# paritybit-ai/XFL

Hardware: AMD Instinct MI355X
Metric: 2048-bit Paillier encrypts/s (device-resident) (higher is better)
Workload: dtype u32; 1 GPU; DJN private-key (CRT) encrypt, obfuscated, precision 7, 1000000 float64 plaintexts/GPU resident in HBM; key_bits=2048, elements_per_gpu=1000000, fixed_base_window_bits=23, fixed_base_window_split=False, parallelism=shard1, table_bytes=193273528320

## Files before the change

### __graft_entry__.py

```python
import os
import sys

ROOT = os.path.dirname(os.path.abspath(__file__))
if ROOT not in sys.path:
    sys.path.insert(0, ROOT)


def build() -> None:
    from xfl_amd import build as b
    b.build()
    from oracle import build as ob
    ob.build()
    import runpy
    try:
        runpy.run_path(os.path.join(ROOT, "tests", "native", "build.py"), run_name="tests_native_build")["build"]()
    except Exception as exc:
        print(f"warning: device self-test harnesses not built: {exc}", file=sys.stderr)
    import xfl_amd
    from xfl_amd import _native
    _native.lib()


def smoke() -> None:
    import numpy as np

    from oracle import paillier_oracle as O
    from xfl_amd import _native as nat
    from xfl_amd.paillier.utils import getprimeover
    import random
    import math

    rng = random.Random(7)
    while True:
        p, q = getprimeover(1024, rng=rng), getprimeover(1024, rng=rng)
        if p != q and math.gcd(p - 1, q - 1) == 2:
            break
    n = p * q
    x = rng.getrandbits(n.bit_length()) | (1 << (n.bit_length() - 1))
    h = pow(-(x * x), n, n * n)
    dk = nat.DeviceKey(2048, n, p, q, h, device=0)
    ok = O.derive_private(p, q, h)
    vals = np.random.default_rng(0).standard_normal(64) * 10
    ms = [O.encode_element(ok, float(v), 7)[0] for v in vals]
    rs = [rng.randrange(1, ok["djn_exp_bound"]) for _ in vals]
    ct = nat.words_to_ints(dk.encrypt_words(nat.ints_to_words(ms, dk.nw), nat.ints_to_words(rs, dk.rand_words)))
    want = [O.encrypt_m(ok, m, r) for m, r in zip(ms, rs)]
    assert ct == want, "HIP encrypt differs from the oracle"
    back = nat.words_to_ints(dk.decrypt_words(nat.ints_to_words(ct, dk.n2w)))
    assert back == ms, "HIP decrypt differs from the oracle"
    print("smoke ok: 64 DJN-CRT encryptions + decryptions bit-exact vs oracle on cuda:0")


if __name__ == "__main__":
    build()
    if "--smoke" in sys.argv:
        smoke()
```

### xfl_amd/csrc/bn_dev.hpp

```cpp
#pragma once
#include <hip/hip_runtime.h>
#include <stdint.h>

namespace xhe {

#define XHE_DEV __device__ __forceinline__
#define XHE_INL __attribute__((always_inline))

#ifndef XHE_SQ_ACC
#define XHE_SQ_ACC 2
#endif
XHE_DEV uint64_t mad64(uint32_t a, uint32_t b, uint64_t c) {
  asm("v_mad_u64_u32 %0, vcc, %1, %2, %0" : "+v"(c) : "v"(a), "v"(b) : "vcc");
  return c;
}
template <int N>
XHE_DEV void mad_shift(uint64_t (&T)[N], const uint32_t (&b)[N], uint32_t a) {
  int j = 1;
#pragma unroll
  for (; j + 6 <= N; j += 6)
    asm("v_mad_u64_u32 %0, vcc, %7, %8, %1\n\t"
        "v_mad_u64_u32 %1, vcc, %7, %9, %2\n\t"
        "v_mad_u64_u32 %2, vcc, %7, %10, %3\n\t"
        "v_mad_u64_u32 %3, vcc, %7, %11, %4\n\t"
// ... 325 lines not shown
    for (int k = 0; k < 8; ++k) nb[0][k] = R.f[k];
    x0 = mad64s(m, R.n0, x0);
    mac4v(T, b, ai, m, 1, R.h);
    advance();
#pragma unroll
    for (int blk = 0; blk < (J8 - 5) / 8; ++blk) {
      const int j = 5 + 8 * blk;
      const int cur = blk & 1;
      if (j + 16 <= J8) {
        asm volatile("" ::"s"(nb[cur][0]), "s"(nb[cur][1]), "s"(nb[cur][2]), "s"(nb[cur][3]), "s"(nb[cur][4]),
                     "s"(nb[cur][5]), "s"(nb[cur][6]), "s"(nb[cur][7]));
        __builtin_amdgcn_sched_barrier(0);
#pragma unroll
        for (int k = 0; k < 8; ++k) nb[cur ^ 1][k] = Np[j + 8 + k];
        __builtin_amdgcn_sched_barrier(0);
      }
      mac8v(T, b, ai, m, j, nb[cur]);
      if (stage < 4) advance();
      else __builtin_amdgcn_sched_barrier(0);
    }
    if constexpr (TL >= 4) mac4v(T, b, ai, m, J8, R.t);
#pragma unroll
    for (int k = (TL >= 4 ? 4 : 0); k < TL; ++k) T[J8 + k - 1] = mad64s(m, R.t[k], mad64(ai, b[J8 + k], T[J8 + k]));
#pragma unroll
    for (int k = 0; k < 4; ++k)
      if (stage < 4) advance();
    T[L - 1] = 0;
    x0 = xn;
    m = mn;
  }

  XHE_DEV void red4v(uint64_t (&T)[L], uint32_t m, int j, const uint32_t* n) const {
    asm("v_mad_u64_u32 %0, vcc, %5, %6, %1\n\t"
        "v_mad_u64_u32 %1, vcc, %5, %7, %2\n\t"
        "v_mad_u64_u32 %2, vcc, %5, %8, %3\n\t"
        "v_mad_u64_u32 %3, vcc, %5, %9, %4"
        : "+v"(T[j - 1]), "+v"(T[j]), "+v"(T[j + 1]), "+v"(T[j + 2])
        : "v"(T[j + 3]), "v"(m), "s"(n[0]), "s"(n[1]), "s"(n[2]), "s"(n[3])
        : "vcc");
  }
  XHE_DEV void red8v(uint64_t (&T)[L], uint32_t m, int j, const uint32_t* n) const {
    asm("v_mad_u64_u32 %0, vcc, %9, %10, %1\n\t"
        "v_mad_u64_u32 %1, vcc, %9, %11, %2\n\t"
        "v_mad_u64_u32 %2, vcc, %9, %12, %3\n\t"
        "v_mad_u64_u32 %3, vcc, %9, %13, %4\n\t"
        "v_mad_u64_u32 %4, vcc, %9, %14, %5\n\t"
        "v_mad_u64_u32 %5, vcc, %9, %15, %6\n\t"
        "v_mad_u64_u32 %6, vcc, %9, %16, %7\n\t"
        "v_mad_u64_u32 %7, vcc, %9, %17, %8"
        : "+v"(T[j - 1]), "+v"(T[j]), "+v"(T[j + 1]), "+v"(T[j + 2]), "+v"(T[j + 3]), "+v"(T[j + 4]),
          "+v"(T[j + 5]), "+v"(T[j + 6])
        : "v"(T[j + 7]), "v"(m), "s"(n[0]), "s"(n[1]), "s"(n[2]), "s"(n[3]), "s"(n[4]), "s"(n[5]), "s"(n[6]),
          "s"(n[7])
        : "vcc");
  }
  XHE_DEV void step1_red(const uint32_t* Np, const NRes& R, uint64_t (&T)[L], uint32_t hi_i, uint32_t& m,
                         uint64_t& x0) const {
    uint64_t xn = 0;
    uint32_t t = 0, mn = 0;
    int stage = 0;
    auto advance = [&]() XHE_INL {
      if (stage == 0) {
        T[0] += x0 >> W;
        asm volatile("" : "+v"(T[0]));
      } else if (stage == 1) {
        xn = T[0];
      } else if (stage == 2) {
        t = (uint32_t)xn * n0inv;
        asm volatile("" : "+v"(t));
      } else if (stage == 3) {
        mn = t & MASK;
        asm volatile("" : "+v"(mn));
      }
      ++stage;
      __builtin_amdgcn_sched_barrier(0);
    };
    uint32_t nb[2][8];
#pragma unroll
    for (int k = 0; k < 8; ++k) nb[0][k] = R.f[k];
    x0 = mad64s(m, R.n0, x0);
    red4v(T, m, 1, R.h);
    advance();
#pragma unroll
    for (int blk = 0; blk < (J8 - 5) / 8; ++blk) {
      const int j = 5 + 8 * blk;
      const int cur = blk & 1;
      if (j + 16 <= J8) {
        asm volatile("" ::"s"(nb[cur][0]), "s"(nb[cur][1]), "s"(nb[cur][2]), "s"(nb[cur][3]), "s"(nb[cur][4]),
                     "s"(nb[cur][5]), "s"(nb[cur][6]), "s"(nb[cur][7]));
        __builtin_amdgcn_sched_barrier(0);
#pragma unroll
        for (int k = 0; k < 8; ++k) nb[cur ^ 1][k] = Np[j + 8 + k];
        __builtin_amdgcn_sched_barrier(0);
      }
      red8v(T, m, j, nb[cur]);
      if (stage < 4) advance();
      else __builtin_amdgcn_sched_barrier(0);
    }
    if constexpr (TL >= 4) red4v(T, m, J8, R.t);
#pragma unroll
    for (int k = (TL >= 4 ? 4 : 0); k < TL; ++k) T[J8 + k - 1] = mad64s(m, R.t[k], T[J8 + k]);
#pragma unroll
    for (int k = 0; k < 4; ++k)
      if (stage < 4) advance();
    T[L - 1] = hi_i;
    x0 = xn;
    m = mn;
  }
  template <int C>
  XHE_DEV uint64_t sq_column(const uint32_t (&a)[L], uint64_t carry) const {
    constexpr int lo = C - (S - 1) > 0 ? C - (S - 1) : 0;
    uint64_t s[XHE_SQ_ACC] = {};
#pragma unroll
    for (int i = lo; 2 * i < C; ++i) s[(i - lo) % XHE_SQ_ACC] = mad64(a[i], a[C - i], s[(i - lo) % XHE_SQ_ACC]);
#pragma unroll
    for (int k = 1; k < XHE_SQ_ACC; ++k) s[0] += s[k];
    uint64_t x = (s[0] << 1) + carry;
    if constexpr ((C & 1) == 0) x = mad64(a[C / 2], a[C / 2], x);
    return x;
  }
  template <int C, class HI>
  XHE_DEV void sq_columns(const uint32_t (&a)[L], uint32_t (&lo)[L], uint64_t carry, uint4& q, const HI& hi) const {
    if constexpr (C < 2 * S) {
      const uint64_t x = C < 2 * S - 1 ? sq_column<C < 2 * S - 1 ? C : 0>(a, carry) : carry;
      const uint32_t limb = (uint32_t)x & MASK;
      if constexpr (C < S) {
        lo[C] = limb;
      } else {
        constexpr int h = C - S;
        if constexpr ((h & 3) == 0) q.x = limb;
        else if constexpr ((h & 3) == 1) q.y = limb;
        else if constexpr ((h & 3) == 2) q.z = limb;
        else q.w = limb;
        if constexpr ((h & 3) == 3 || C == 2 * S - 1) {
          if constexpr ((h & 3) < 3) q.w = 0;
          if constexpr ((h & 3) < 2) q.z = 0;
          if constexpr ((h & 3) < 1) q.y = 0;
          hi.put4(h >> 2, q);
        }
      }
      sq_columns<C + 1, HI>(a, lo, x >> W, q, hi);
    }
  }
  static constexpr bool kSqr = TPI == 1 && L >= 13;
  template <class HI>
  XHE_DEV void sqr(uint32_t (&b)[L], const HI& hi) const {
    uint32_t lo[L];
    uint4 q = make_uint4(0u, 0u, 0u, 0u);
    sq_columns<0, HI>(b, lo, 0ull, q, hi);
    uint64_t T[L];
#pragma unroll
    for (int j = 0; j < L; ++j) T[j] = lo[j];
    hi.sync();
    const uint32_t* Np = np();
    NRes R;
    load_res(Np, R);
    uint64_t x0 = T[0];
    uint32_t m = ((uint32_t)x0 * n0inv) & MASK;
    uint4 cur = hi.load4(0);
    int i = 0;
    for (; i + 4 <= S; i += 4) {
      uint4 nxt = hi.load4(i + 4 < S4 ? i + 4 : i);
      __builtin_amdgcn_sched_barrier(0);
      step1_red(Np, R, T, cur.x, m, x0);
      __builtin_amdgcn_sched_barrier(0);
      step1_red(Np, R, T, cur.y, m, x0);
      __builtin_amdgcn_sched_barrier(0);
      step1_red(Np, R, T, cur.z, m, x0);
      __builtin_amdgcn_sched_barrier(0);
      step1_red(Np, R, T, cur.w, m, x0);
      __builtin_amdgcn_sched_barrier(0);
      cur = nxt;
    }
#pragma unroll
    for (int r = 0; r < (S & 3); ++r) step1_red(Np, R, T, comp4(cur, r), m, x0);
    normalize(T, b);
  }

  XHE_DEV void step(const uint32_t* Np, uint64_t (&T)[L], const uint32_t (&b)[L], uint32_t ai, uint32_t ai_next,
                    uint32_t& m, uint64_t& x0, bool lead) const {
    static_assert(L >= 5, "pipelined step needs L >= 5");
    uint64_t xn = 0;
    uint32_t t = 0, mn = 0;
    int stage = 0;
    auto advance = [&]() XHE_INL {
      if (stage == 0) {
        T[0] += x0 >> W;
        asm volatile("" : "+v"(T[0]));
      } else if (stage == 1) {
        xn = mad64(ai_next, b[0], T[0]);
        asm volatile("" : "+v"(xn));
      } else if (stage == 2) {
        t = (uint32_t)xn * n0inv;
        asm volatile("" : "+v"(t));
      } else if (stage == 3) {
        mn = G::bcast0(t & MASK);
        asm volatile("" : "+v"(mn));
      }
      ++stage;
      __builtin_amdgcn_sched_barrier(0);
    };
    x0 = madN(Np, m, 0, x0);
    mac4(Np, T, b, ai, m, 1);
    advance();
    int j = 5;
#pragma unroll
    for (; j + 8 <= L; j += 8) {
      mac8(Np, T, b, ai, m, j);
      if (stage < 4) advance();
    }
#pragma unroll
    for (; j + 4 <= L; j += 4) {
      mac4(Np, T, b, ai, m, j);
      if (stage < 4) advance();
    }
#pragma unroll
    for (; j < L; ++j) T[j - 1] = madN(Np, m, j, mad64(ai, b[j], T[j]));
#pragma unroll
    for (int k = 0; k < 4; ++k)
      if (stage < 4) advance();
    T[L - 1] = (uint64_t)G::from_next((uint32_t)x0 & MASK);
    x0 = xn;
    m = mn;
  }

  XHE_DEV void normalize(const uint64_t (&T)[L], uint32_t (&b)[L]) const {
    uint64_t c = 0;
#pragma unroll
    for (int j = 0; j < L; ++j) {
      uint64_t x = T[j] + c;
      b[j] = (uint32_t)x & MASK;
      c = x >> W;
      __builtin_amdgcn_sched_barrier(0);
    }
    if constexpr (TPI >= 4) {
      uint64_t cin = G::from_prev64(c);
      uint32_t all = 1u;
#pragma unroll
      for (int j = 0; j < L; ++j) {
        uint64_t x = (uint64_t)b[j] + cin;
        b[j] = (uint32_t)x & MASK;
        cin = x >> W;
        all &= (b[j] == MASK) ? 1u : 0u;
        __builtin_amdgcn_sched_barrier(0);
      }
      constexpr uint64_t top = TPI == 16 ? 0x8000800080008000ull : TPI == 8 ? 0x8080808080808080ull
                                                                            : 0x8888888888888888ull;
      const uint64_t gm = __builtin_amdgcn_ballot_w64(cin != 0) & ~top;
      const uint64_t tm = (gm | __builtin_amdgcn_ballot_w64(all != 0)) & ~top;
      const uint64_t cm = (gm + tm) ^ gm ^ tm;
      uint32_t ci = (uint32_t)(cm >> (threadIdx.x & 63)) & 1u;
#pragma unroll
      for (int j = 0; j < L; ++j) {
        uint32_t x = b[j] + ci;
        b[j] = x & MASK;
        ci = x >> W;
      }
    } else if constexpr (TPI > 1) {
#pragma unroll
      for (int r = 1; r < TPI; ++r) {
        uint64_t cin = G::from_prev64(c);
#pragma unroll
        for (int j = 0; j < L; ++j) {
          uint64_t x = (uint64_t)b[j] + cin;
          b[j] = (uint32_t)x & MASK;
          cin = x >> W;
          __builtin_amdgcn_sched_barrier(0);
        }
        c = cin;
      }
    }
  }

  template <class A>
  XHE_DEV void mul(uint32_t (&b)[L], const A& a) const {
    uint64_t T[L];
#pragma unroll
    for (int j = 0; j < L; ++j) T[j] = 0;
    run<A>(T, b, a);
    normalize(T, b);
  }

  template <class A>
  XHE_DEV void run(uint64_t (&T)[L], const uint32_t (&b)[L], const A& a) const {
    const bool lead = G::g() == 0;
    const uint32_t* Np = np();
    uint4 cur = a.load4(0);
    uint64_t x0 = mad64(cur.x, b[0], T[0]);
    uint32_t m = G::bcast0(((uint32_t)x0 * n0inv) & MASK);
    int i = 0;
    if constexpr (TPI == 1 && L >= 13) {
      NRes R;
      load_res(Np, R);
      for (; i + 4 <= S; i += 4) {
        uint4 nxt = a.load4(i + 4 < S4 ? i + 4 : i);
        __builtin_amdgcn_sched_barrier(0);
        step1(Np, R, T, b, cur.x, cur.y, m, x0, lead);
        __builtin_amdgcn_sched_barrier(0);
        step1(Np, R, T, b, cur.y, cur.z, m, x0, lead);
        __builtin_amdgcn_sched_barrier(0);
        step1(Np, R, T, b, cur.z, cur.w, m, x0, lead);
        __builtin_amdgcn_sched_barrier(0);
        step1(Np, R, T, b, cur.w, nxt.x, m, x0, lead);
        __builtin_amdgcn_sched_barrier(0);
        cur = nxt;
      }
#pragma unroll
      for (int r = 0; r < (S & 3); ++r)
        step1(Np, R, T, b, comp4(cur, r), r + 1 < (S & 3) ? comp4(cur, r + 1) : 0u, m, x0, lead);
      return;
    }
    for (; i + 4 <= S; i += 4) {
      uint4 nxt = a.load4(i + 4 < S4 ? i + 4 : i);
      __builtin_amdgcn_sched_barrier(0);
      step(Np, T, b, cur.x, cur.y, m, x0, lead);
      __builtin_amdgcn_sched_barrier(0);
      step(Np, T, b, cur.y, cur.z, m, x0, lead);
      __builtin_amdgcn_sched_barrier(0);
      step(Np, T, b, cur.z, cur.w, m, x0, lead);
      __builtin_amdgcn_sched_barrier(0);
      step(Np, T, b, cur.w, nxt.x, m, x0, lead);
      __builtin_amdgcn_sched_barrier(0);
      cur = nxt;
    }
#pragma unroll
    for (int r = 0; r < (S & 3); ++r)
      step(Np, T, b, comp4(cur, r), r + 1 < (S & 3) ? comp4(cur, r + 1) : 0u, m, x0, lead);
  }

  template <class A>
  XHE_DEV void redc_wide(uint32_t (&b)[L], const A& hi) const {
    uint64_t T[L];
#pragma unroll
    for (int j = 0; j < L; ++j) T[j] = b[j];
    const bool lead = G::g() == 0;
    const bool last = G::g() == TPI - 1;
    const uint32_t* Np = np();
    for (int i0 = 0; i0 < S4; i0 += 4) {
      uint4 h4 = hi.load4(i0);
#pragma unroll
      for (int r = 0; r < 4; ++r) {
        if (i0 + r < S) {
          uint64_t x0 = T[0];
          uint32_t m = ((uint32_t)x0 * n0inv) & MASK;
          m = G::bcast0(m);
          x0 = madN(Np, m, 0, x0);
#pragma unroll
          for (int j = 1; j < L; ++j) T[j - 1] = madN(Np, m, j, T[j]);
          uint64_t up = G::from_next64(x0);
          T[L - 1] = last ? (uint64_t)comp4(h4, r) : up;
          T[0] += lead ? (x0 >> W) : 0ull;
        }
      }
    }
    normalize(T, b);
  }

  XHE_DEV void reduce_once(uint32_t (&b)[L]) const {
    uint32_t d[L];
    uint32_t br = 0;
    const uint32_t* Np = np();
#pragma unroll
    for (int j = 0; j < L; ++j) {
      int64_t x = (int64_t)b[j] - (int64_t)nj(Np, j) - (int64_t)br;
      br = x < 0 ? 1u : 0u;
      d[j] = (uint32_t)(x + ((int64_t)br << W));
    }
    if constexpr (TPI > 1) {
      uint32_t total = br;
#pragma unroll
      for (int r = 1; r < TPI; ++r) {
        uint32_t bin = G::from_prev(br);
#pragma unroll
        for (int j = 0; j < L; ++j) {
          int64_t x = (int64_t)d[j] - (int64_t)bin;
          bin = x < 0 ? 1u : 0u;
          d[j] = (uint32_t)(x + ((int64_t)bin << W));
        }
        br = bin;
        total |= bin;
      }
      br = G::bcast_last(total);
    }
    if (!br) {
#pragma unroll
      for (int j = 0; j < L; ++j) b[j] = d[j];
    }
  }

  XHE_DEV void add_sub_rows(uint32_t (&b)[L], const uint32_t* add, const uint32_t* subp, int sub_stride) const {
    const int g = G::g();
    int64_t c = 0;
#pragma unroll
    for (int j = 0; j < L; ++j) {
      int64_t x = (int64_t)b[j] + (int64_t)add[g * L + j] - (int64_t)subp[(size_t)(g * L + j) * sub_stride] + c;
      c = x >> W;
      b[j] = (uint32_t)(x & MASK);
    }
    if constexpr (TPI > 1) {
#pragma unroll
      for (int r = 1; r < TPI; ++r) {
        int64_t cin = (int64_t)G::from_prev64((uint64_t)c);
#pragma unroll
        for (int j = 0; j < L; ++j) {
          int64_t x = (int64_t)b[j] + cin;
          cin = x >> W;
          b[j] = (uint32_t)(x & MASK);
        }
        c = cin;
      }
    }
  }

  XHE_DEV void add_row(uint32_t (&b)[L], const uint32_t* row) const {
    const int g = G::g();
    uint64_t T[L];
#pragma unroll
    for (int j = 0; j < L; ++j) T[j] = (uint64_t)b[j] + row[g * L + j];
    normalize(T, b);
  }

  template <class A>
  XHE_DEV void wide_mul_add_store(const uint32_t (&b)[L], const A& a, uint32_t* ws, int stride,
                                  uint32_t* __restrict__ out, int nwords) const {
    const int g = G::g();
    const bool lead = g == 0;
    uint64_t T[L];
#pragma unroll
    for (int j = 0; j < L; ++j) T[j] = ws[(size_t)(g * L + j) * stride];
    wave_sync_mem_();
    for (int i0 = 0; i0 < S4; i0 += 4) {
      uint4 a4 = a.load4(i0);
#pragma unroll
      for (int r = 0; r < 4; ++r) {
        if (i0 + r < S) {
          uint32_t ai = comp4(a4, r);
          uint64_t x0 = mad64(ai, b[0], T[0]);
          if (lead) ws[(size_t)(i0 + r) * stride] = (uint32_t)x0 & MASK;
          mad_shift(T, b, ai);
          T[L - 1] = G::from_next64(x0);
          T[0] += lead ? (x0 >> W) : 0ull;
        }
      }
    }
    uint32_t hi[L];
    normalize(T, hi);
#pragma unroll
    for (int j = 0; j < L; ++j) ws[(size_t)(S + g * L + j) * stride] = hi[j];
    wave_sync_mem_();
    if (out) pack_words_<W, TPI>(ws, stride, 2 * S, out, nwords);
  }

  template <int GG>
  XHE_DEV void load_words_g(uint32_t (&b)[L], const uint32_t* __restrict__ w, int nwords) const {
#pragma unroll
    for (int j = 0; j < L; ++j) {
      const int bit = W * (GG * L + j);
      const int k = bit >> 5, sh = bit & 31;
      const uint32_t lo = word_or0(w, k, nwords);
      const uint32_t hi = sh + W > 32 ? word_or0(w, k + 1, nwords) : 0u;
      b[j] = (uint32_t)((((uint64_t)hi << 32) | lo) >> sh) & MASK;
    }
  }
  template <int GG>
  XHE_DEV void load_words_from(uint32_t (&b)[L], const uint32_t* __restrict__ w, int nwords, int g) const {
    if constexpr (GG == TPI - 1) {
      load_words_g<GG>(b, w, nwords);
    } else {
      if (g == GG) load_words_g<GG>(b, w, nwords);
      else load_words_from<GG + 1>(b, w, nwords, g);
    }
  }
  XHE_DEV void load_words(uint32_t (&b)[L], const uint32_t* __restrict__ w, int nwords) const {
    load_words_from<0>(b, w, nwords, G::g());
  }
  XHE_DEV void store_strided_n(const uint32_t (&b)[L], uint32_t* p, int stride, int nlimbs) const {
    p = opaque(p);
    const int g = G::g();
#pragma unroll
    for (int j = 0; j < L; ++j)
      if (g * L + j < nlimbs) p[(size_t)(g * L + j) * stride] = b[j];
  }
  XHE_DEV void store_words(const uint32_t (&b)[L], uint32_t* __restrict__ out, int nwords) const {
    constexpr int LB = L * W;
    constexpr int NWM = (LB + 31) / 32 + 1;
    const uint32_t n0 = G::from_next(b[0]);
    const uint32_t n1 = G::from_next(L > 1 ? b[1] : 0u);
// ... 46 lines not shown
```

### xfl_amd/csrc/pdigit_dev.hpp

```cpp
#pragma once
#include "bn_dev.hpp"

namespace xhe {

struct PmdLdsQ {
  const uint32_t* q;
  XHE_DEV uint4 load4(int i) const { return *reinterpret_cast<const uint4*>(q + (i >> 2) * 256); }
};

template <int K_>
struct PMD {
  static constexpr int K = K_, W = 28, BL = 6;
  static constexpr int NQ = (2 * K + 3) / 4;
  static constexpr uint32_t MASK = (1u << W) - 1u;
  static_assert((K - 1) % BL == 0, "positions 1..K-1 in blocks of 6");
  static_assert((double)(3 * K + 2) * (double)(1ull << 57) < 18446744073709551616.0, "accumulator bound");

  uint32_t p[K];
  uint32_t n0inv;

  XHE_DEV void init(const uint32_t* __restrict__ P, uint32_t ninv) {
#pragma unroll
    for (int j = 0; j < K; ++j) p[j] = __builtin_amdgcn_readfirstlane(P[j]);
    n0inv = ninv;
// ... 49 lines not shown
        "v_mad_u64_u32 %9, vcc, %14, %27, %10\n\t"
        "v_mad_u64_u32 %10, vcc, %14, %28, %11\n\t"
        "v_mad_u64_u32 %11, vcc, %14, %29, %13\n\t"
        "v_mad_u64_u32 %0, vcc, %16, %30, %0\n\t"
        "v_mad_u64_u32 %1, vcc, %16, %31, %1\n\t"
        "v_mad_u64_u32 %2, vcc, %16, %32, %2\n\t"
        "v_mad_u64_u32 %3, vcc, %16, %33, %3\n\t"
        "v_mad_u64_u32 %4, vcc, %16, %34, %4\n\t"
        "v_mad_u64_u32 %5, vcc, %16, %35, %5\n\t"
        "v_mad_u64_u32 %6, vcc, %15, %18, %6\n\t"
        "v_mad_u64_u32 %7, vcc, %15, %19, %7\n\t"
        "v_mad_u64_u32 %8, vcc, %15, %20, %8\n\t"
        "v_mad_u64_u32 %9, vcc, %15, %21, %9\n\t"
        "v_mad_u64_u32 %10, vcc, %15, %22, %10\n\t"
        "v_mad_u64_u32 %11, vcc, %15, %23, %11\n\t"
        "v_mad_u64_u32 %6, vcc, %17, %30, %6\n\t"
        "v_mad_u64_u32 %7, vcc, %17, %31, %7\n\t"
        "v_mad_u64_u32 %8, vcc, %17, %32, %8\n\t"
        "v_mad_u64_u32 %9, vcc, %17, %33, %9\n\t"
        "v_mad_u64_u32 %10, vcc, %17, %34, %10\n\t"
        "v_mad_u64_u32 %11, vcc, %17, %35, %11"
          : "+v"(T1[j - 1]), "+v"(T1[j]), "+v"(T1[j + 1]), "+v"(T1[j + 2]), "+v"(T1[j + 3]), "+v"(T1[j + 4]),
            "+v"(T2[j - 1]), "+v"(T2[j]), "+v"(T2[j + 1]), "+v"(T2[j + 2]), "+v"(T2[j + 3]), "+v"(T2[j + 4])
          : "v"(T1[j + 5]), "v"(T2[j + 5]), "v"(e), "v"(f), "v"(m1), "v"(m2), "v"(a[j]), "v"(a[j + 1]),
            "v"(a[j + 2]), "v"(a[j + 3]), "v"(a[j + 4]), "v"(a[j + 5]), "v"(c[j]), "v"(c[j + 1]), "v"(c[j + 2]),
            "v"(c[j + 3]), "v"(c[j + 4]), "v"(c[j + 5]), "s"(p[j]), "s"(p[j + 1]), "s"(p[j + 2]), "s"(p[j + 3]),
            "s"(p[j + 4]), "s"(p[j + 5])
          : "vcc");
    }
  }

  template <bool SQ = false>
  XHE_DEV void step(uint64_t (&T1)[K], uint64_t (&T2)[K], const uint32_t (&a)[K], const uint32_t (&c)[K],
                    uint32_t e, uint32_t f, uint32_t en, uint32_t fn, uint32_t& m1, uint32_t& m2, uint64_t& x1,
                    uint64_t& x2, uint32_t topc) const {
    uint64_t x1n = 0, x2n = 0;
    uint32_t t1 = 0, t2 = 0, m1n = 0, m2n = 0;
    asm("v_mad_u64_u32 %0, vcc, %2, %4, %0\n\t"
        "v_mad_u64_u32 %1, vcc, %3, %4, %1"
        : "+v"(x1), "+v"(x2)
        : "v"(m1), "v"(m2), "s"(p[0])
        : "vcc");
#pragma unroll
    for (int b = 0; b < (K - 1) / BL; ++b) {
      const int j = 1 + BL * b;
      blk12<SQ>(T1, T2, a, c, e, SQ ? (e << 1) : f, m1, m2, j);
      if (b == 0) {
        T1[0] += x1 >> W;
        T2[0] += x2 >> W;
        asm volatile("" : "+v"(T1[0]), "+v"(T2[0]));
      } else if (b == 1) {
        if constexpr (SQ) {
          asm("v_mad_u64_u32 %0, vcc, %2, %3, %5\n\t"
              "v_mad_u64_u32 %1, vcc, %4, %7, %6"
              : "=&v"(x1n), "=v"(x2n)
              : "v"(en), "v"(a[0]), "v"(en << 1), "v"(T1[0]), "v"(T2[0]), "v"(c[0])
              : "vcc");
        } else {
          asm("v_mad_u64_u32 %0, vcc, %2, %4, %6\n\t"
              "v_mad_u64_u32 %1, vcc, %2, %5, %7\n\t"
              "v_mad_u64_u32 %1, vcc, %3, %4, %1"
              : "=&v"(x1n), "=&v"(x2n)
              : "v"(en), "v"(fn), "v"(a[0]), "v"(c[0]), "v"(T1[0]), "v"(T2[0])
              : "vcc");
        }
        asm volatile("" : "+v"(x1n), "+v"(x2n));
      } else if (b == 2) {
        t1 = (uint32_t)x1n * n0inv;
        t2 = (uint32_t)x2n * n0inv;
        asm volatile("" : "+v"(t1), "+v"(t2));
      } else if (b == 3) {
        m1n = t1 & MASK;
        m2n = t2 & MASK;
        asm volatile("" : "+v"(m1n), "+v"(m2n));
      }
      __builtin_amdgcn_sched_barrier(0);
    }
    T1[K - 1] = 0;
    T2[K - 1] = (uint64_t)(topc - m1);
    x1 = x1n;
    x2 = x2n;
    m1 = m1n;
    m2 = m2n;
  }

  XHE_DEV void mul(uint32_t (&a)[K], uint32_t (&c)[K], const uint32_t* slot, const uint32_t* topc) const {
    run<false>(a, c, slot, topc);
  }
  XHE_DEV void sqr(uint32_t (&a)[K], uint32_t (&c)[K], const uint32_t* slot, const uint32_t* topc) const {
    run<true>(a, c, slot, topc);
  }
  template <bool SQ>
  XHE_DEV void run(uint32_t (&a)[K], uint32_t (&c)[K], const uint32_t* slot, const uint32_t* topc) const {
    uint64_t T1[K], T2[K];
#pragma unroll
    for (int j = 0; j < K; ++j) T1[j] = T2[j] = 0;
    uint2 p0 = *reinterpret_cast<const uint2*>(slot);
    uint64_t x1 = mad64(p0.x, a[0], 0ull);
    uint64_t x2 = SQ ? mad64(p0.x << 1, c[0], 0ull) : mad64(p0.y, a[0], mad64(p0.x, c[0], 0ull));
    uint32_t m1 = ((uint32_t)x1 * n0inv) & MASK, m2 = ((uint32_t)x2 * n0inv) & MASK;
    for (int q = 0; q < K / 2; ++q) {
      const uint32_t* sq = slot + q * 256;
      const uint2 tc = *reinterpret_cast<const uint2*>(topc + 2 * q);
      const uint2 p1 = *reinterpret_cast<const uint2*>(sq + 2);
      __builtin_amdgcn_sched_barrier(0);
      step<SQ>(T1, T2, a, c, p0.x, p0.y, p1.x, p1.y, m1, m2, x1, x2, tc.x);
      __builtin_amdgcn_sched_barrier(0);
      p0 = *reinterpret_cast<const uint2*>(sq + 256);
      __builtin_amdgcn_sched_barrier(0);
      step<SQ>(T1, T2, a, c, p1.x, p1.y, p0.x, p0.y, m1, m2, x1, x2, tc.y);
      __builtin_amdgcn_sched_barrier(0);
    }
    if constexpr (K & 1) step<SQ>(T1, T2, a, c, p0.x, p0.y, 0u, 0u, m1, m2, x1, x2, topc[K - 1]);
    normalize(T1, a);
    normalize(T2, c);
  }

  XHE_DEV void blk12_row(uint64_t (&T1)[K], uint64_t (&T2)[K], const uint32_t (&a)[K], const uint32_t (&c)[K],
                         uint32_t e, uint32_t m1, uint32_t m2, int j) const {
    asm(
      "v_mad_u64_u32 %0, vcc, %14, %17, %1\n\t"
      "v_mad_u64_u32 %1, vcc, %14, %18, %2\n\t"
      "v_mad_u64_u32 %2, vcc, %14, %19, %3\n\t"
      "v_mad_u64_u32 %3, vcc, %14, %20, %4\n\t"
      "v_mad_u64_u32 %4, vcc, %14, %21, %5\n\t"
      "v_mad_u64_u32 %5, vcc, %14, %22, %12\n\t"
      "v_mad_u64_u32 %6, vcc, %14, %23, %7\n\t"
      "v_mad_u64_u32 %7, vcc, %14, %24, %8\n\t"
      "v_mad_u64_u32 %8, vcc, %14, %25, %9\n\t"
      "v_mad_u64_u32 %9, vcc, %14, %26, %10\n\t"
      "v_mad_u64_u32 %10, vcc, %14, %27, %11\n\t"
      "v_mad_u64_u32 %11, vcc, %14, %28, %13\n\t"
      "v_mad_u64_u32 %0, vcc, %15, %29, %0\n\t"
      "v_mad_u64_u32 %1, vcc, %15, %30, %1\n\t"
      "v_mad_u64_u32 %2, vcc, %15, %31, %2\n\t"
      "v_mad_u64_u32 %3, vcc, %15, %32, %3\n\t"
      "v_mad_u64_u32 %4, vcc, %15, %33, %4\n\t"
      "v_mad_u64_u32 %5, vcc, %15, %34, %5\n\t"
      "v_mad_u64_u32 %6, vcc, %16, %29, %6\n\t"
      "v_mad_u64_u32 %7, vcc, %16, %30, %7\n\t"
      "v_mad_u64_u32 %8, vcc, %16, %31, %8\n\t"
      "v_mad_u64_u32 %9, vcc, %16, %32, %9\n\t"
      "v_mad_u64_u32 %10, vcc, %16, %33, %10\n\t"
      "v_mad_u64_u32 %11, vcc, %16, %34, %11"
        : "+v"(T1[j - 1]), "+v"(T1[j]), "+v"(T1[j + 1]), "+v"(T1[j + 2]), "+v"(T1[j + 3]), "+v"(T1[j + 4]),
          "+v"(T2[j - 1]), "+v"(T2[j]), "+v"(T2[j + 1]), "+v"(T2[j + 2]), "+v"(T2[j + 3]), "+v"(T2[j + 4])
        : "v"(T1[j + 5]), "v"(T2[j + 5]), "v"(e), "v"(m1), "v"(m2), "v"(a[j]), "v"(a[j + 1]), "v"(a[j + 2]),
          "v"(a[j + 3]), "v"(a[j + 4]), "v"(a[j + 5]), "v"(c[j]), "v"(c[j + 1]), "v"(c[j + 2]), "v"(c[j + 3]),
          "v"(c[j + 4]), "v"(c[j + 5]), "s"(p[j]), "s"(p[j + 1]), "s"(p[j + 2]), "s"(p[j + 3]), "s"(p[j + 4]),
          "s"(p[j + 5])
        : "vcc");
  }

  XHE_DEV void step_row(uint64_t (&T1)[K], uint64_t (&T2)[K], const uint32_t (&a)[K], const uint32_t (&c)[K],
                        uint32_t e, uint32_t en, uint32_t& m1, uint32_t& m2, uint64_t& x1, uint64_t& x2,
                        uint32_t topc) const {
    uint64_t x1n = 0, x2n = 0;
    uint32_t t1 = 0, t2 = 0, m1n = 0, m2n = 0;
    asm("v_mad_u64_u32 %0, vcc, %2, %4, %0\n\t"
        "v_mad_u64_u32 %1, vcc, %3, %4, %1"
        : "+v"(x1), "+v"(x2)
        : "v"(m1), "v"(m2), "s"(p[0])
        : "vcc");
#pragma unroll
    for (int b = 0; b < (K - 1) / BL; ++b) {
      const int j = 1 + BL * b;
      blk12_row(T1, T2, a, c, e, m1, m2, j);
      if (b == 0) {
        T1[0] += x1 >> W;
        T2[0] += x2 >> W;
        asm volatile("" : "+v"(T1[0]), "+v"(T2[0]));
      } else if (b == 1) {
        asm("v_mad_u64_u32 %0, vcc, %2, %3, %5\n\t"
            "v_mad_u64_u32 %1, vcc, %2, %4, %6"
            : "=&v"(x1n), "=&v"(x2n)
            : "v"(en), "v"(a[0]), "v"(c[0]), "v"(T1[0]), "v"(T2[0])
            : "vcc");
        asm volatile("" : "+v"(x1n), "+v"(x2n));
      } else if (b == 2) {
        t1 = (uint32_t)x1n * n0inv;
        t2 = (uint32_t)x2n * n0inv;
        asm volatile("" : "+v"(t1), "+v"(t2));
      } else if (b == 3) {
        m1n = t1 & MASK;
        m2n = t2 & MASK;
        asm volatile("" : "+v"(m1n), "+v"(m2n));
      }
      __builtin_amdgcn_sched_barrier(0);
    }
    T1[K - 1] = 0;
    T2[K - 1] = (uint64_t)(topc - m1);
    x1 = x1n;
    x2 = x2n;
    m1 = m1n;
    m2 = m2n;
  }

  XHE_DEV void mul_row(uint32_t (&a)[K], uint32_t (&c)[K], const uint32_t* slot, const uint32_t* topc) const {
    uint64_t T1[K], T2[K];
#pragma unroll
    for (int j = 0; j < K; ++j) T1[j] = T2[j] = 0;
    uint2 p0 = *reinterpret_cast<const uint2*>(slot);
    uint64_t x1 = mad64(p0.x, a[0], 0ull);
    uint64_t x2 = mad64(p0.x, c[0], 0ull);
    uint32_t m1 = ((uint32_t)x1 * n0inv) & MASK, m2 = ((uint32_t)x2 * n0inv) & MASK;
    for (int h = 0; h < K / 2; ++h) {
      const int k = 2 * h + 2;
      const uint2 tc = *reinterpret_cast<const uint2*>(topc + 2 * h);
      const uint2 p1 = *reinterpret_cast<const uint2*>(slot + (k >> 2) * 256 + (k & 2));
      __builtin_amdgcn_sched_barrier(0);
      step_row(T1, T2, a, c, p0.x, p0.y, m1, m2, x1, x2, tc.x);
      __builtin_amdgcn_sched_barrier(0);
      step_row(T1, T2, a, c, p0.y, p1.x, m1, m2, x1, x2, tc.y);
      __builtin_amdgcn_sched_barrier(0);
      p0 = p1;
    }
    if constexpr (K & 1) step_row(T1, T2, a, c, p0.x, 0u, m1, m2, x1, x2, topc[K - 1]);
    normalize(T1, a);
    normalize(T2, c);
  }

  static constexpr int EQ = (K + 3) / 4;
  static constexpr int LW = (W * K + 31) / 32;
  static_assert(EQ + (LW + 3) / 4 <= NQ, "e limbs and the log sum share the slot of an interleaved row");

  XHE_DEV static void lam_zero(uint32_t* slot) {
#pragma unroll
    for (int q = 0; q < (LW + 3) / 4; ++q) *reinterpret_cast<uint4*>(slot + (EQ + q) * 256) = make_uint4(0u, 0u, 0u, 0u);
  }
  template <int HW>
  XHE_DEV static void lam_add(uint32_t* slot, const uint32_t (&lam)[HW]) {
    constexpr int LQ = (LW + 3) / 4;
    static_assert(HW >= 1 && HW <= 4 * LQ, "at most a whole sum");
    uint32_t s[4 * LQ];
#pragma unroll
    for (int q = 0; q < LQ; ++q) {
      const uint4 v = *reinterpret_cast<const uint4*>(slot + (EQ + q) * 256);
      s[4 * q] = v.x, s[4 * q + 1] = v.y, s[4 * q + 2] = v.z, s[4 * q + 3] = v.w;
    }
    uint32_t cy = 0;
#pragma unroll
    for (int k = 0; k < LW; ++k) {
      const uint64_t x = (uint64_t)s[k] + (k < HW ? lam[k] : 0u) + cy;
      s[k] = (uint32_t)x;
      cy = (uint32_t)(x >> 32);
    }
#pragma unroll
    for (int q = 0; q < LQ; ++q)
      *reinterpret_cast<uint4*>(slot + (EQ + q) * 256) = make_uint4(s[4 * q], s[4 * q + 1], s[4 * q + 2], s[4 * q + 3]);
  }
  XHE_DEV static void lam_add_slot(uint32_t* slot, const uint32_t* other) {
    constexpr int LQ = (LW + 3) / 4;
    uint32_t o[4 * LQ];
#pragma unroll
    for (int q = 0; q < LQ; ++q) {
      const uint4 v = *reinterpret_cast<const uint4*>(other + (EQ + q) * 256);
      o[4 * q] = v.x, o[4 * q + 1] = v.y, o[4 * q + 2] = v.z, o[4 * q + 3] = v.w;
    }
    lam_add<4 * LQ>(slot, o);
  }

  XHE_DEV void finish(const uint32_t (&a)[K], uint32_t (&c)[K], uint32_t* slot, const uint32_t* Pl) const {
    constexpr int LQ = (LW + 3) / 4;
    {
      uint32_t s[4 * LQ + 1];
#pragma unroll
      for (int q = 0; q < LQ; ++q) {
        const uint4 v = *reinterpret_cast<const uint4*>(slot + (EQ + q) * 256);
        s[4 * q] = v.x, s[4 * q + 1] = v.y, s[4 * q + 2] = v.z, s[4 * q + 3] = v.w;
      }
      s[4 * LQ] = 0u;
      auto limb = [&](int i) -> uint32_t {
        const int bit = W * i, k = bit >> 5, sh = bit & 31;
        return i < K ? (__builtin_amdgcn_alignbit(k + 1 < LW ? s[k + 1] : 0u, s[k], sh) & MASK) : 0u;
      };
#pragma unroll
      for (int q = 0; q < EQ; ++q)
        *reinterpret_cast<uint4*>(slot + q * 256) = make_uint4(limb(4 * q), limb(4 * q + 1), limb(4 * q + 2), limb(4 * q + 3));
    }
    __builtin_amdgcn_sched_barrier(0);
    uint32_t t[K];
#pragma unroll
    for (int j = 0; j < K; ++j) t[j] = a[j];
    Mont<K, W, 1> MN;
    MN.init(Pl, n0inv);
    MN.mul(t, PmdLdsQ{slot});
    uint32_t cy = 0;
#pragma unroll
    for (int j = 0; j < K; ++j) {
      const uint32_t x = c[j] + t[j] + cy;
      c[j] = j + 1 < K ? (x & MASK) : x;
      cy = j + 1 < K ? (x >> W) : 0u;
    }
  }

  XHE_DEV static void normalize(const uint64_t (&T)[K], uint32_t (&b)[K]) {
    uint64_t cy = 0;
#pragma unroll
    for (int j = 0; j < K; ++j) {
      const uint64_t x = T[j] + cy;
      b[j] = j + 1 < K ? ((uint32_t)x & MASK) : (uint32_t)x;
      cy = x >> W;
      __builtin_amdgcn_sched_barrier(0);
    }
  }

  XHE_DEV void to_mont2(const uint32_t (&a)[K], const uint32_t (&c)[K], uint32_t (&x)[2 * K]) const {
    uint64_t T[2 * K];
#pragma unroll
    for (int j = 0; j < K; ++j) {
      T[j] = 0;
      T[K + j] = a[j];
    }
#pragma unroll
    for (int i = 0; i < K; ++i) {
#pragma unroll
      for (int j = 0; j < K; ++j) T[i + j] = mad64s(c[j], p[i], T[i + j]);
    }
    uint64_t cy = 0;
#pragma unroll
    for (int j = 0; j < 2 * K; ++j) {
      const uint64_t v = T[j] + cy;
      x[j] = j + 1 < 2 * K ? ((uint32_t)v & MASK) : (uint32_t)v;
      cy = v >> W;
    }
  }
};

template <int K>
XHE_DEV void pmd_redc_wide(const PMD<K>& M, uint64_t (&T)[2 * K], uint32_t (&t)[K], uint32_t (&m)[K]) {
  constexpr uint32_t MASK = PMD<K>::MASK;
  uint64_t cy = 0;
#pragma unroll
  for (int i = 0; i < K; ++i) {
    uint64_t x = T[i] + cy;
    const uint32_t mi = ((uint32_t)x * M.n0inv) & MASK;
    m[i] = mi;
    x = mad64s(mi, M.p[0], x);
    cy = x >> 28;
#pragma unroll
    for (int j = 1; j < K; ++j) T[i + j] = mad64s(mi, M.p[j], T[i + j]);
    __builtin_amdgcn_sched_barrier(0);
  }
#pragma unroll
  for (int j = 0; j < K; ++j) {
    const uint64_t x = T[K + j] + cy;
    t[j] = j + 1 < K ? ((uint32_t)x & MASK) : (uint32_t)x;
    cy = x >> 28;
  }
}

template <int K>
XHE_DEV void pmd_lam_plain(const PMD<K>& M, uint32_t* slot, const uint32_t* __restrict__ mw, int nw,
                           const uint32_t* mu, const uint32_t* Pl) {
  using D = PMD<K>;
  constexpr int LQ = (D::LW + 3) / 4;
  uint32_t t[K];
  {
    uint64_t T[2 * K];
#pragma unroll
    for (int j = 0; j < 2 * K; ++j) {
      const int bit = 28 * j, k = bit >> 5, sh = bit & 31;
      const uint32_t lo = word_or0(mw, k, nw);
      const uint32_t hi = sh + 28 > 32 ? word_or0(mw, k + 1, nw) : 0u;
      T[j] = (uint32_t)((((uint64_t)hi << 32) | lo) >> sh) & D::MASK;
    }
    uint32_t q[K];
    pmd_redc_wide<K>(M, T, t, q);
  }
  __builtin_amdgcn_sched_barrier(0);
  Mont<K, 28, 1> MN;
  MN.init(Pl, M.n0inv);
  MN.mul(t, ARow{mu});
  uint32_t s[4 * LQ];
#pragma unroll
  for (int k = 0; k < 4 * LQ; ++k) {
    const int bit = 32 * k, j = bit / 28, sh = bit - 28 * j;
    uint64_t v = j < K ? (uint64_t)t[j] : 0ull;
    if (j + 1 < K) v |= (uint64_t)t[j + 1] << 28;
    if (j + 2 < K) v |= (uint64_t)t[j + 2] << 56;
    s[k] = k < D::LW ? (uint32_t)(v >> sh) : 0u;
  }
#pragma unroll
  for (int q = 0; q < LQ; ++q)
    *reinterpret_cast<uint4*>(slot + (D::EQ + q) * 256) = make_uint4(s[4 * q], s[4 * q + 1], s[4 * q + 2], s[4 * q + 3]);
}

template <int K>
XHE_DEV uint32_t pmd_sub(uint32_t (&r)[K], const uint32_t (&s)[K]) {
  int64_t br = 0;
#pragma unroll
  for (int j = 0; j < K; ++j) {
    const int64_t v = (int64_t)r[j] - (int64_t)s[j] + br;
    r[j] = (uint32_t)v & ((1u << 28) - 1u);
    br = v >> 28;
  }
  return br ? 1u : 0u;
}

template <int K>
XHE_DEV bool pmd_csub(const PMD<K>& M, uint32_t (&r)[K]) {
  int64_t br = 0;
#pragma unroll
  for (int j = 0; j < K; ++j) br = ((int64_t)r[j] - (int64_t)M.p[j] + br) >> 28;
  const bool ge = br == 0;
  br = 0;
#pragma unroll
  for (int j = 0; j < K; ++j) {
    const int64_t v = (int64_t)r[j] - (int64_t)(ge ? M.p[j] : 0u) + br;
    r[j] = (uint32_t)v & ((1u << 28) - 1u);
    br = v >> 28;
  }
  return ge;
}

template <int K>
XHE_DEV void pmd_mod_small(const PMD<K>& M, uint32_t (&m)[K]) {
  constexpr uint32_t MASK = PMD<K>::MASK;
  const uint32_t mt = (m[K - 1] << 4) | (m[K - 2] >> 24);
  const uint32_t pt = (M.p[K - 1] << 4) | (M.p[K - 2] >> 24);
  const uint32_t q = mt / (pt + 1u);
  uint64_t cy = 0;
  int64_t br = 0;
#pragma unroll
  for (int j = 0; j < K; ++j) {
    const uint64_t qp = (uint64_t)q * M.p[j] + cy;
    cy = qp >> 28;
    const int64_t v = (int64_t)m[j] - (int64_t)(qp & MASK) + br;
    m[j] = (uint32_t)v & MASK;
    br = v >> 28;
  }
#pragma unroll
  for (int t = 0; t < 3; ++t) pmd_csub<K>(M, m);
}

template <int K>
XHE_DEV void pmd_from_mont2(const PMD<K>& M, const uint32_t (&X)[2 * K], const uint32_t* RmodP, uint32_t (&e)[K],
                            uint32_t (&f)[K]) {
  uint32_t m[K];
  {
    uint64_t T[2 * K];
#pragma unroll
    for (int j = 0; j < 2 * K; ++j) T[j] = X[j];
    pmd_redc_wide<K>(M, T, e, m);
  }
  __builtin_amdgcn_sched_barrier(0);
  const bool ge = pmd_csub<K>(M, e);
  __builtin_amdgcn_sched_barrier(0);
  pmd_mod_small<K>(M, m);
  __builtin_amdgcn_sched_barrier(0);
  int64_t br = 0;
#pragma unroll
  for (int j = 0; j < K; ++j) {
    const int64_t v = (int64_t)(ge ? RmodP[j] : 0u) - (int64_t)m[j] + br;
    f[j] = (uint32_t)v & ((1u << 28) - 1u);
    br = v >> 28;
  }
  if (br) {
    int64_t cy = 0;
#pragma unroll
    for (int j = 0; j < K; ++j) {
      const int64_t v = (int64_t)f[j] + (int64_t)M.p[j] + cy;
      f[j] = (uint32_t)v & ((1u << 28) - 1u);
      cy = v >> 28;
    }
  }
}

template <int K, int RW>
XHE_DEV void unpack_pairs_lds(uint32_t* slot) {
  constexpr int HW = RW / 2;
  uint32_t w[RW];
#pragma unroll
  for (int q = 0; q < RW / 4; ++q) {
    const uint4 v = *reinterpret_cast<const uint4*>(slot + q * 256);
    w[4 * q] = v.x;
    w[4 * q + 1] = v.y;
    w[4 * q + 2] = v.z;
    w[4 * q + 3] = v.w;
  }
  auto limb = [&](int base, int i) -> uint32_t {
    const int bit = 28 * i, k = bit >> 5, sh = bit & 31;
    const uint32_t lo = k < HW ? w[base + k] : 0u, hi = k + 1 < HW ? w[base + k + 1] : 0u;
    return i < K ? (__builtin_amdgcn_alignbit(hi, lo, sh) & ((1u << 28) - 1u)) : 0u;
  };
#pragma unroll
  for (int q = 0; q < (2 * K + 3) / 4; ++q)
    *reinterpret_cast<uint4*>(slot + q * 256) =
        make_uint4(limb(0, 2 * q), limb(HW, 2 * q), limb(0, 2 * q + 1), limb(HW, 2 * q + 1));
}

template <int K, int HW>
XHE_DEV void unpack_e_lds(uint32_t* slot) {
  static_assert(HW % 4 == 0 && 32 * HW >= 28 * K - 27, "the packed digit holds K limbs");
  uint32_t w[HW];
#pragma unroll
  for (int q = 0; q < HW / 4; ++q) {
    const uint4 v = *reinterpret_cast<const uint4*>(slot + q * 256);
    w[4 * q] = v.x;
    w[4 * q + 1] = v.y;
    w[4 * q + 2] = v.z;
    w[4 * q + 3] = v.w;
  }
  auto limb = [&](int i) -> uint32_t {
    const int bit = 28 * i, k = bit >> 5, sh = bit & 31;
    const uint32_t lo = k < HW ? w[k] : 0u, hi = k + 1 < HW ? w[k + 1] : 0u;
    return i < K ? (__builtin_amdgcn_alignbit(hi, lo, sh) & ((1u << 28) - 1u)) : 0u;
  };
#pragma unroll
  for (int q = 0; q < (K + 3) / 4; ++q)
    *reinterpret_cast<uint4*>(slot + q * 256) = make_uint4(limb(4 * q), limb(4 * q + 1), limb(4 * q + 2), limb(4 * q + 3));
}

}

namespace xhe {

struct OpLds {
  const uint2* p;
  int stride;
  XHE_DEV uint2 load(int i) const { return p[i * stride]; }
};
struct OpRow {
  const uint2* __restrict__ p;
  XHE_DEV uint2 load(int i) const { return p[i]; }
// ... 591 lines not shown
```

Before: 49.51 million encrypts/s.

## Stream wide REDC high limbs through LDS and peel first PMD multiply row

The wide Montgomery reduction in pmd_lam_plain no longer holds a 2K-entry 64-bit array in registers. It now writes the upper limbs into the LDS slot and reuses the single-thread square's pipelined row reducer (red_rows) through redc_wide. mul_row peels off the first step with a variant that writes its products directly, which removes the zero initialisation of T1/T2. lam_add replaces its scalar carry loop with chained add-with-carry inline assembly. The intent is lower register pressure and fewer instructions, at the cost of extra LDS traffic and more hand-written assembly.

After: 51.05 million encrypts/s, median of 6. +3.1%, better.

```diff
diff --git a/__graft_entry__.py b/__graft_entry__.py
--- a/__graft_entry__.py
+++ b/__graft_entry__.py
@@ -12,10 +12,11 @@
     from oracle import build as ob
     ob.build()
     import runpy
-    try:
-        runpy.run_path(os.path.join(ROOT, "tests", "native", "build.py"), run_name="tests_native_build")["build"]()
-    except Exception as exc:
-        print(f"warning: device self-test harnesses not built: {exc}", file=sys.stderr)
+    for script in ("build.py", "build_redc_block.py"):
+        try:
+            runpy.run_path(os.path.join(ROOT, "tests", "native", script), run_name="tests_native_build")["build"]()
+        except Exception as exc:
+            print(f"warning: device self-test harnesses not built ({script}): {exc}", file=sys.stderr)
     import xfl_amd
     from xfl_amd import _native
     _native.lib()
diff --git a/xfl_amd/csrc/bn_dev.hpp b/xfl_amd/csrc/bn_dev.hpp
--- a/xfl_amd/csrc/bn_dev.hpp
+++ b/xfl_amd/csrc/bn_dev.hpp
@@ -501,6 +501,11 @@
 #pragma unroll
     for (int j = 0; j < L; ++j) T[j] = lo[j];
     hi.sync();
+    red_rows(T, hi);
+    normalize(T, b);
+  }
+  template <class HI>
+  XHE_DEV void red_rows(uint64_t (&T)[L], const HI& hi) const {
     const uint32_t* Np = np();
     NRes R;
     load_res(Np, R);
@@ -523,7 +528,6 @@
     }
 #pragma unroll
     for (int r = 0; r < (S & 3); ++r) step1_red(Np, R, T, comp4(cur, r), m, x0);
-    normalize(T, b);
   }
 
   XHE_DEV void step(const uint32_t* Np, uint64_t (&T)[L], const uint32_t (&b)[L], uint32_t ai, uint32_t ai_next,
@@ -682,6 +686,11 @@
     uint64_t T[L];
 #pragma unroll
     for (int j = 0; j < L; ++j) T[j] = b[j];
+    if constexpr (TPI == 1 && L >= 13) {
+      red_rows(T, hi);
+      normalize(T, b);
+      return;
+    }
     const bool lead = G::g() == 0;
     const bool last = G::g() == TPI - 1;
     const uint32_t* Np = np();
diff --git a/xfl_amd/csrc/pdigit_dev.hpp b/xfl_amd/csrc/pdigit_dev.hpp
--- a/xfl_amd/csrc/pdigit_dev.hpp
+++ b/xfl_amd/csrc/pdigit_dev.hpp
@@ -225,6 +225,42 @@
         : "vcc");
   }
 
+  XHE_DEV void blk12_row0(uint64_t (&T1)[K], uint64_t (&T2)[K], const uint32_t (&a)[K], const uint32_t (&c)[K],
+                          uint32_t e, uint32_t m1, uint32_t m2, int j) const {
+    asm(
+      "v_mad_u64_u32 %0, vcc, %12, %15, 0\n\t"
+      "v_mad_u64_u32 %1, vcc, %12, %16, 0\n\t"
+      "v_mad_u64_u32 %2, vcc, %12, %17, 0\n\t"
+      "v_mad_u64_u32 %3, vcc, %12, %18, 0\n\t"
+      "v_mad_u64_u32 %4, vcc, %12, %19, 0\n\t"
+      "v_mad_u64_u32 %5, vcc, %12, %20, 0\n\t"
+      "v_mad_u64_u32 %6, vcc, %12, %21, 0\n\t"
+      "v_mad_u64_u32 %7, vcc, %12, %22, 0\n\t"
+      "v_mad_u64_u32 %8, vcc, %12, %23, 0\n\t"
+      "v_mad_u64_u32 %9, vcc, %12, %24, 0\n\t"
+      "v_mad_u64_u32 %10, vcc, %12, %25, 0\n\t"
+      "v_mad_u64_u32 %11, vcc, %12, %26, 0\n\t"
+      "v_mad_u64_u32 %0, vcc, %13, %27, %0\n\t"
+      "v_mad_u64_u32 %1, vcc, %13, %28, %1\n\t"
+      "v_mad_u64_u32 %2, vcc, %13, %29, %2\n\t"
+      "v_mad_u64_u32 %3, vcc, %13, %30, %3\n\t"
+      "v_mad_u64_u32 %4, vcc, %13, %31, %4\n\t"
+      "v_mad_u64_u32 %5, vcc, %13, %32, %5\n\t"
+      "v_mad_u64_u32 %6, vcc, %14, %27, %6\n\t"
+      "v_mad_u64_u32 %7, vcc, %14, %28, %7\n\t"
+      "v_mad_u64_u32 %8, vcc, %14, %29, %8\n\t"
+      "v_mad_u64_u32 %9, vcc, %14, %30, %9\n\t"
+      "v_mad_u64_u32 %10, vcc, %14, %31, %10\n\t"
+      "v_mad_u64_u32 %11, vcc, %14, %32, %11"
+        : "=&v"(T1[j - 1]), "=&v"(T1[j]), "=&v"(T1[j + 1]), "=&v"(T1[j + 2]), "=&v"(T1[j + 3]), "=&v"(T1[j + 4]),
+          "=&v"(T2[j - 1]), "=&v"(T2[j]), "=&v"(T2[j + 1]), "=&v"(T2[j + 2]), "=&v"(T2[j + 3]), "=&v"(T2[j + 4])
+        : "v"(e), "v"(m1), "v"(m2), "v"(a[j]), "v"(a[j + 1]), "v"(a[j + 2]), "v"(a[j + 3]), "v"(a[j + 4]),
+          "v"(a[j + 5]), "v"(c[j]), "v"(c[j + 1]), "v"(c[j + 2]), "v"(c[j + 3]), "v"(c[j + 4]), "v"(c[j + 5]),
+          "s"(p[j]), "s"(p[j + 1]), "s"(p[j + 2]), "s"(p[j + 3]), "s"(p[j + 4]), "s"(p[j + 5])
+        : "vcc");
+  }
+
+  template <bool FIRST = false>
   XHE_DEV void step_row(uint64_t (&T1)[K], uint64_t (&T2)[K], const uint32_t (&a)[K], const uint32_t (&c)[K],
                         uint32_t e, uint32_t en, uint32_t& m1, uint32_t& m2, uint64_t& x1, uint64_t& x2,
                         uint32_t topc) const {
@@ -238,7 +274,8 @@
 #pragma unroll
     for (int b = 0; b < (K - 1) / BL; ++b) {
       const int j = 1 + BL * b;
-      blk12_row(T1, T2, a, c, e, m1, m2, j);
+      if constexpr (FIRST) blk12_row0(T1, T2, a, c, e, m1, m2, j);
+      else blk12_row(T1, T2, a, c, e, m1, m2, j);
       if (b == 0) {
         T1[0] += x1 >> W;
         T2[0] += x2 >> W;
@@ -270,25 +307,24 @@
   }
 
   XHE_DEV void mul_row(uint32_t (&a)[K], uint32_t (&c)[K], const uint32_t* slot, const uint32_t* topc) const {
+    static_assert(K & 1, "the first step alone, then pairs of steps");
     uint64_t T1[K], T2[K];
-#pragma unroll
-    for (int j = 0; j < K; ++j) T1[j] = T2[j] = 0;
     uint2 p0 = *reinterpret_cast<const uint2*>(slot);
     uint64_t x1 = mad64(p0.x, a[0], 0ull);
     uint64_t x2 = mad64(p0.x, c[0], 0ull);
     uint32_t m1 = ((uint32_t)x1 * n0inv) & MASK, m2 = ((uint32_t)x2 * n0inv) & MASK;
+    step_row<true>(T1, T2, a, c, p0.x, p0.y, m1, m2, x1, x2, topc[0]);
     for (int h = 0; h < K / 2; ++h) {
       const int k = 2 * h + 2;
-      const uint2 tc = *reinterpret_cast<const uint2*>(topc + 2 * h);
+      const uint32_t tc1 = topc[2 * h + 1], tc2 = topc[2 * h + 2];
       const uint2 p1 = *reinterpret_cast<const uint2*>(slot + (k >> 2) * 256 + (k & 2));
       __builtin_amdgcn_sched_barrier(0);
-      step_row(T1, T2, a, c, p0.x, p0.y, m1, m2, x1, x2, tc.x);
-      __builtin_amdgcn_sched_barrier(0);
-      step_row(T1, T2, a, c, p0.y, p1.x, m1, m2, x1, x2, tc.y);
+      step_row(T1, T2, a, c, p0.y, p1.x, m1, m2, x1, x2, tc1);
+      __builtin_amdgcn_sched_barrier(0);
+      step_row(T1, T2, a, c, p1.x, p1.y, m1, m2, x1, x2, tc2);
       __builtin_amdgcn_sched_barrier(0);
       p0 = p1;
     }
-    if constexpr (K & 1) step_row(T1, T2, a, c, p0.x, 0u, m1, m2, x1, x2, topc[K - 1]);
     normalize(T1, a);
     normalize(T2, c);
   }
@@ -301,23 +337,58 @@
 #pragma unroll
     for (int q = 0; q < (LW + 3) / 4; ++q) *reinterpret_cast<uint4*>(slot + (EQ + q) * 256) = make_uint4(0u, 0u, 0u, 0u);
   }
+  template <bool FIRST, int NS, int NL>
+  XHE_DEV static void add8(uint32_t (&s)[NS], const uint32_t (&l)[NL], int k, uint64_t& cy) {
+    if constexpr (FIRST) {
+      asm("v_add_co_u32 %0, vcc, %0, %9\n\t"
+          "v_addc_co_u32 %1, vcc, %1, %10, vcc\n\t"
+          "v_addc_co_u32 %2, vcc, %2, %11, vcc\n\t"
+          "v_addc_co_u32 %3, vcc, %3, %12, vcc\n\t"
+          "v_addc_co_u32 %4, vcc, %4, %13, vcc\n\t"
+          "v_addc_co_u32 %5, vcc, %5, %14, vcc\n\t"
+          "v_addc_co_u32 %6, vcc, %6, %15, vcc\n\t"
+          "v_addc_co_u32_e64 %7, %8, %7, %16, vcc"
+          : "+v"(s[k]), "+v"(s[k + 1]), "+v"(s[k + 2]), "+v"(s[k + 3]), "+v"(s[k + 4]), "+v"(s[k + 5]),
+            "+v"(s[k + 6]), "+v"(s[k + 7]), "=s"(cy)
+          : "v"(l[k]), "v"(l[k + 1]), "v"(l[k + 2]), "v"(l[k + 3]), "v"(l[k + 4]), "v"(l[k + 5]), "v"(l[k + 6]),
+            "v"(l[k + 7])
+          : "vcc");
+    } else {
+      asm("v_addc_co_u32_e64 %0, vcc, %0, %9, %8\n\t"
+          "v_addc_co_u32 %1, vcc, %1, %10, vcc\n\t"
+          "v_addc_co_u32 %2, vcc, %2, %11, vcc\n\t"
+          "v_addc_co_u32 %3, vcc, %3, %12, vcc\n\t"
+          "v_addc_co_u32 %4, vcc, %4, %13, vcc\n\t"
+          "v_addc_co_u32 %5, vcc, %5, %14, vcc\n\t"
+          "v_addc_co_u32 %6, vcc, %6, %15, vcc\n\t"
+          "v_addc_co_u32_e64 %7, %8, %7, %16, vcc"
+          : "+v"(s[k]), "+v"(s[k + 1]), "+v"(s[k + 2]), "+v"(s[k + 3]), "+v"(s[k + 4]), "+v"(s[k + 5]),
+            "+v"(s[k + 6]), "+v"(s[k + 7]), "+s"(cy)
+          : "v"(l[k]), "v"(l[k + 1]), "v"(l[k + 2]), "v"(l[k + 3]), "v"(l[k + 4]), "v"(l[k + 5]), "v"(l[k + 6]),
+            "v"(l[k + 7])
+          : "vcc");
+    }
+  }
   template <int HW>
   XHE_DEV static void lam_add(uint32_t* slot, const uint32_t (&lam)[HW]) {
     constexpr int LQ = (LW + 3) / 4;
-    static_assert(HW >= 1 && HW <= 4 * LQ, "at most a whole sum");
+    constexpr int NW = HW < LW ? HW : LW;
+    static_assert(HW >= 8 && HW <= 4 * LQ, "at least one block of the chain, at most a whole sum");
     uint32_t s[4 * LQ];
 #pragma unroll
     for (int q = 0; q < LQ; ++q) {
       const uint4 v = *reinterpret_cast<const uint4*>(slot + (EQ + q) * 256);
       s[4 * q] = v.x, s[4 * q + 1] = v.y, s[4 * q + 2] = v.z, s[4 * q + 3] = v.w;
     }
-    uint32_t cy = 0;
-#pragma unroll
-    for (int k = 0; k < LW; ++k) {
-      const uint64_t x = (uint64_t)s[k] + (k < HW ? lam[k] : 0u) + cy;
-      s[k] = (uint32_t)x;
-      cy = (uint32_t)(x >> 32);
-    }
+    uint64_t cy;
+    add8<true>(s, lam, 0, cy);
+#pragma unroll
+    for (int k = 8; k + 8 <= NW; k += 8) add8<false>(s, lam, k, cy);
+#pragma unroll
+    for (int k = NW & ~7; k < NW; ++k)
+      asm("v_addc_co_u32_e64 %0, %1, %0, %2, %1" : "+v"(s[k]), "+s"(cy) : "v"(lam[k]));
+#pragma unroll
+    for (int k = NW; k < LW; ++k) asm("v_addc_co_u32_e64 %0, %1, 0, %0, %1" : "+v"(s[k]), "+s"(cy));
 #pragma unroll
     for (int q = 0; q < LQ; ++q)
       *reinterpret_cast<uint4*>(slot + (EQ + q) * 256) = make_uint4(s[4 * q], s[4 * q + 1], s[4 * q + 2], s[4 * q + 3]);
@@ -424,26 +495,35 @@
 }
 
 template <int K>
+XHE_DEV void pmd_redc_words(const Mont<K, 28, 1>& MN, uint32_t* slot, const uint32_t* __restrict__ mw, int nw,
+                            uint32_t (&t)[K]) {
+  constexpr uint32_t MASK = PMD<K>::MASK;
+  auto limb = [&](int j) -> uint32_t {
+    const int bit = 28 * j, k = bit >> 5, sh = bit & 31;
+    const uint32_t lo = word_or0(mw, k, nw);
+    const uint32_t hi = sh + 28 > 32 ? word_or0(mw, k + 1, nw) : 0u;
+    return j < 2 * K ? (uint32_t)((((uint64_t)hi << 32) | lo) >> sh) & MASK : 0u;
+  };
+#pragma unroll
+  for (int q = 0; q < PMD<K>::EQ; ++q)
+    *reinterpret_cast<uint4*>(slot + q * 256) =
+        make_uint4(limb(K + 4 * q), limb(K + 4 * q + 1), limb(K + 4 * q + 2), limb(K + 4 * q + 3));
+#pragma unroll
+  for (int j = 0; j < K; ++j) t[j] = limb(j);
+  __builtin_amdgcn_sched_barrier(0);
+  MN.redc_wide(t, PmdLdsQ{slot});
+}
+
+template <int K>
 XHE_DEV void pmd_lam_plain(const PMD<K>& M, uint32_t* slot, const uint32_t* __restrict__ mw, int nw,
                            const uint32_t* mu, const uint32_t* Pl) {
   using D = PMD<K>;
   constexpr int LQ = (D::LW + 3) / 4;
-  uint32_t t[K];
-  {
-    uint64_t T[2 * K];
-#pragma unroll
-    for (int j = 0; j < 2 * K; ++j) {
-      const int bit = 28 * j, k = bit >> 5, sh = bit & 31;
-      const uint32_t lo = word_or0(mw, k, nw);
-      const uint32_t hi = sh + 28 > 32 ? word_or0(mw, k + 1, nw) : 0u;
-      T[j] = (uint32_t)((((uint64_t)hi << 32) | lo) >> sh) & D::MASK;
-    }
-    uint32_t q[K];
-    pmd_redc_wide<K>(M, T, t, q);
-  }
-  __builtin_amdgcn_sched_barrier(0);
   Mont<K, 28, 1> MN;
   MN.init(Pl, M.n0inv);
+  uint32_t t[K];
+  pmd_redc_words<K>(MN, slot, mw, nw, t);
+  __builtin_amdgcn_sched_barrier(0);
   MN.mul(t, ARow{mu});
   uint32_t s[4 * LQ];
 #pragma unroll
```
